# mjevans26/Satellite_ComputerVision

Hardware: AMD Instinct MI355X
Metric: tiles/sec (train) 256x256x4 U-Net (higher is better)
Workload: dtype bf16; 1 GPU; U-Net 256x256x4 bfloat16 training, batch 64 per GPU (BASELINE configs[1]); global_batch=64, parallelism=dp1, loss=weighted_categorical_crossentropy, optimizer=adam(9e-4)

## Files before the change

### include/satcv.h

```cpp
#ifndef SATCV_H
#define SATCV_H
#include <stdint.h>
#ifdef __cplusplus
extern "C" {
#endif

typedef double satcv_stat_t;

enum { SATCV_OK = 0, SATCV_ERR_INVALID = -1, SATCV_ERR_HIP = -2, SATCV_ERR_UNSUPPORTED = -3 };
enum { SATCV_F32 = 0, SATCV_BF16 = 1,
       SATCV_FP8 = 2 ,
       SATCV_FP8X = 3 ,
       SATCV_F64 = 4  };
#define SATCV_STAT_ROWS 32

const char* satcv_version(void);
const char* satcv_last_error(void);
int satcv_device_info(int32_t* out4);

int satcv_ingest_nhwc(const float* src, void* dst, int64_t npix, int32_t c, int32_t cpad,
                      int32_t dtype, void* stream);
int satcv_ingest_nhwc_scaled(const float* src, void* dst, int64_t npix, int32_t c, int32_t cpad, float mul, int32_t dtype, void* stream);
int satcv_ingest_chw(const void* src, int32_t src_kind, float scale, void* dst, int32_t n,
                     int32_t c, int32_t h, int32_t w, int32_t cpad, int32_t dtype, void* stream);
// ... 104 lines not shown
  const float* in_scale; const float* in_shift; int32_t in_relu;
  const void* w_dgrad;
  void* dx; int32_t lddx;
  float* dw; int32_t cin, cout;
  int32_t n, h, w_;
  int32_t kh, kw, dil;
  float* workspace; int64_t workspace_bytes;
  int32_t dtype;
  int32_t accumulate;
  satcv_stat_t* bst_sums; int32_t bst_sums_ld;
  const float* bst_mean; const float* bst_rstd;
  int32_t bst_act_form;
  const void* dpool; int32_t lddp; const void* amax;
  const float* hg_dlogits; const float* hg_w; int32_t hg_ncls;
  int32_t defer_reduce;
} satcv_bwdf_desc;
int64_t satcv_conv2d_bwd_fused_workspace(const satcv_bwdf_desc* d);
int satcv_conv2d_bwd_fused(const satcv_bwdf_desc* d, void* stream);
int satcv_conv2d_bwd_fused_reduce_job(const satcv_bwdf_desc* d, satcv_reduce_job* job);

typedef struct satcv_bwdf_plan_info {
  int32_t cin, cout, nw, wps, pool, nodg, cins, hg;
  int32_t bst, pad_;
  int64_t tiles, workgroups, tiles_min, tiles_max, lds_bytes, ws_bytes;
} satcv_bwdf_plan_info;
int satcv_conv2d_bwd_fused_plan_info(const satcv_bwdf_desc* d, int32_t ncu, satcv_bwdf_plan_info* info);

typedef struct satcv_ctbf_desc {
  const void* g; int32_t ldg;
  const void* yup; int32_t ldy;
// ... 385 lines not shown
```

### satellite_computervision_amd/_lib.py

```python
import ctypes as C
import os

import torch

from . import switches

_HERE = os.path.dirname(os.path.abspath(__file__))
LIB_PATH = switches.read('lib') or os.path.join(_HERE, 'libsatcv.so')

F32, BF16, FP8, FP8X, F64 = 0, 1, 2, 3, 4
STAT_ROWS = 32
COMPOSITE_MAX_T = 256

c_i32, c_i64, c_f32, c_vp = C.c_int32, C.c_int64, C.c_float, C.c_void_p


class ConvDesc(C.Structure):
    _fields_ = [('x0', c_vp), ('x1', c_vp), ('c0', c_i32), ('c1', c_i32),
                ('in_scale', c_vp), ('in_shift', c_vp), ('in_relu', c_i32),
                ('w', c_vp), ('bias', c_vp), ('y', c_vp), ('ldy', c_i32),
                ('stats', c_vp), ('stats_ld', c_i32),
                ('n', c_i32), ('h', c_i32), ('w_', c_i32),
                ('cout', c_i32), ('cout_pad', c_i32),
                ('kh', c_i32), ('kw', c_i32), ('dil', c_i32),
# ... 132 lines not shown
                   'ws': ('cin', 'nt', 'wps', 'wn', 'dil'), 'tr': ('cin', 'cout', 'th'),
                   'convt_thin': ('cin', 'cout', 'nw', 'wps', 'nsplit'), 'convt_thin_dgrad': ('cin', 'cout', 'nw', 'wps')}


class BwdfDesc(C.Structure):
    _fields_ = [('g', c_vp), ('yraw', c_vp), ('ldg', c_i32),
                ('bn_scale', c_vp), ('bn_shift', c_vp), ('bn_mean', c_vp), ('bn_rstd', c_vp), ('bn_coef', c_vp), ('linear', c_i32),
                ('x0', c_vp), ('x1', c_vp), ('c0', c_i32), ('c1', c_i32),
                ('in_scale', c_vp), ('in_shift', c_vp), ('in_relu', c_i32),
                ('w_dgrad', c_vp), ('dx', c_vp), ('lddx', c_i32),
                ('dw', c_vp), ('cin', c_i32), ('cout', c_i32),
                ('n', c_i32), ('h', c_i32), ('w_', c_i32), ('kh', c_i32), ('kw', c_i32), ('dil', c_i32),
                ('workspace', c_vp), ('workspace_bytes', c_i64), ('dtype', c_i32), ('accumulate', c_i32),
                ('bst_sums', c_vp), ('bst_sums_ld', c_i32), ('bst_mean', c_vp), ('bst_rstd', c_vp), ('bst_act_form', c_i32),
                ('dpool', c_vp), ('lddp', c_i32), ('amax', c_vp),
                ('hg_dlogits', c_vp), ('hg_w', c_vp), ('hg_ncls', c_i32), ('defer_reduce', c_i32)]


class CtbfDesc(C.Structure):
    _fields_ = [('g', c_vp), ('ldg', c_i32), ('yup', c_vp), ('ldy', c_i32),
                ('bn_scale', c_vp), ('bn_shift', c_vp), ('bn_mean', c_vp), ('bn_rstd', c_vp), ('bn_c1', c_vp), ('bn_c2', c_vp), ('linear', c_i32),
                ('x', c_vp), ('ldx', c_i32), ('in_scale', c_vp), ('in_shift', c_vp), ('in_relu', c_i32),
                ('w_dgrad', c_vp), ('w_npad', c_i32), ('dx', c_vp), ('lddx', c_i32), ('dw', c_vp), ('cin', c_i32), ('cout', c_i32),
                ('n', c_i32), ('h', c_i32), ('w_', c_i32), ('f', c_i32), ('workspace', c_vp), ('workspace_bytes', c_i64),
                ('dtype', c_i32), ('accumulate', c_i32), ('defer_reduce', c_i32),
                ('bst_sums', c_vp), ('bst_sums_ld', c_i32), ('bst_mean', c_vp), ('bst_rstd', c_vp)]


class BwdfPlanInfo(C.Structure):
    _fields_ = [(k, c_i32) for k in ('cin', 'cout', 'nw', 'wps', 'pool', 'nodg', 'cins', 'hg', 'bst', 'pad_')] + \
               [(k, c_i64) for k in ('tiles', 'workgroups', 'tiles_min', 'tiles_max', 'lds_bytes', 'ws_bytes')]
# ... 216 lines not shown
```

### satellite_computervision_amd/csrc/conv_bwd_fused.hip

```cpp
#include "igemm_common.hpp"
#include <cstdlib>
#include <cstring>

#ifndef BWDF_ABL
#define BWDF_ABL 0
#endif
#define FABL(bit) ((BWDF_ABL & (bit)) != 0)

int wgrad_reduce_slabs(const float* ws, float* dw, int nslab, int taps, int kpad, int npad, int cin, int nvalid, int accumulate, hipStream_t st);
void reduce_job_fill(satcv_reduce_job* job, const float* ws, float* dw, int nslab, int taps, int kpad, int npad, int cin, int nvalid, int transposed, int accumulate);
void satcv_prof_begin(int kind, double flops, hipStream_t st);
void satcv_prof_end(int kind, hipStream_t st);

struct BwdfArgs {
  IgemmArgs e;
  const void* g; const void* yraw; int ldg;
  const float* bn_scale; const float* bn_shift; const float* bn_mean; const float* bn_rstd; const float* bn_coef; int bn_c, linear;
  const void* x0; const void* x1; int c0, c1;
  const float* in_scale; const float* in_shift; int in_relu;
  const void* w;
  float* ws;
  int tiles_x, tiles_y;
  satcv_stat_t* bst_sums; int bst_ld; const float* bst_mean; const float* bst_rstd;
  int bst_act_form;
  const void* dp; int lddp; const unsigned char* amax;
  const float* hg_dl; const float* hg_w;
};

__device__ __forceinline__ bf16x4 tr_read4(const bf16* p) {
  short4v v = __builtin_amdgcn_ds_read_tr16_b64_v4i16((__attribute__((address_space(3))) short4v*)(p));
  return __builtin_bit_cast(bf16x4, v);
}

constexpr bool bwdf_carries_sums(bool nodg, int wps, bool pool) { return !nodg && (wps != 1 || pool); }

template <int CIN, int COUT, int NW, int WPS, bool POOL = false, bool NODG = false, int CINS = CIN, bool HG = false>
__global__ __launch_bounds__(NW * 64, WPS) void bwd_fused_kernel(const BwdfArgs a, const int total_tiles) {
  static_assert(!HG || !POOL, "the head feeds a decoder block");
  typedef bf16 T;
  constexpr int TW = 32, TH = 8, BM = 256, RL = TH + 2, CL = TW + 2, PITCH = CL, EL = 8, NTHREADS = NW * 64;
  constexpr int SD = COUT / 8, SX = CIN / 8, SXR = CINS / 8;
// ... 354 lines not shown
    }
    if (POOL && t + 1 < t_hi) issue_pool(n0, y0, x0);
    __syncthreads();
    {
      constexpr int OPITCH = CIN + 8, VPR = CIN / 8;
      T* ldsO = reinterpret_cast<T*>(smem_raw + O_OFF);
      T* op = ldsO + ((wave * MT) * 32 + 4 * hh) * OPITCH + r;
#pragma unroll
      for (int m = 0; m < MT; ++m)
#pragma unroll
        for (int n = 0; n < NT; ++n)
#pragma unroll
          for (int i = 0; i < 16; ++i) op[(m * 32 + (i & 3) + 8 * (i >> 2)) * OPITCH + n * 32] = (T)acc[m][n][i];
      __syncthreads();
      const int vq = tid % VPR;
      T* yp = reinterpret_cast<T*>(a.e.y) + ((size_t)(tn0 * a.e.h + ty0) * a.e.w_ + tx0) * a.e.ldy + vq * 8;
      const unsigned row_pitch = (unsigned)a.e.w_ * a.e.ldy;
      const T* xact = ldsX + vq * XSTRIDE;
#pragma unroll 2
      for (int it = tid; it < BM * VPR; it += NTHREADS) {
        const int q = it / VPR;
        const uint4 dv = *reinterpret_cast<const uint4*>(ldsO + q * OPITCH + vq * 8);
        if constexpr (!FABL(4)) *reinterpret_cast<uint4*>(yp + (size_t)((q / TW) * row_pitch + (q % TW) * (unsigned)a.e.ldy)) = dv;
        else asm volatile("" :: "v"(dv.x));
        if (BST && a.bst_sums) {
          const bf16x8 d8 = __builtin_bit_cast(bf16x8, dv);
          const bf16x8 a8 = *reinterpret_cast<const bf16x8*>(xact + q * EL);
#pragma unroll
          for (int e = 0; e < 8; ++e) {
            const float df = (float)d8[e], af = (float)a8[e];
            bs1[e] += af > 0.f ? df : 0.f;
            bs2[e] += df * af;
          }
        }
      }
    }
    }
    __syncthreads();
// ... 74 lines not shown
  long long grid = (long long)ncu * per_cu;
  if (grid > total) grid = total;
  return (int)grid;
}

static bool bwdf_shape_ok(const satcv_bwdf_desc* d, int& cin_s) {
  cin_s = d->c0 + d->c1;
  if (d->dtype != SATCV_BF16 || d->kh != 3 || d->kw != 3 || d->dil != 1) return false;
  if (d->n <= 0 || d->h <= 0 || d->w_ <= 0 || !satcv_pixels_ok(d->n, d->h, d->w_, 1)) return false;
  if (d->x1 && d->c0 % 8 != 0) return false;
  if (d->h % 8 != 0 || d->w_ % 32 != 0) return false;
  if (d->ldg % 8 != 0 || ((uintptr_t)d->g % 16) != 0 || ((uintptr_t)d->yraw % 16) != 0) return false;
  if (d->hg_dlogits && (!d->hg_w || d->hg_ncls != 2 || d->dpool || ((uintptr_t)d->hg_dlogits % 8) != 0)) return false;
  if (d->dx && (d->lddx % 8 != 0 || ((uintptr_t)d->dx % 16) != 0)) return false;
  if ((long long)d->w_ * d->ldg >= (1 << 23)) return false;
  if (d->dpool) {
    if (!d->amax || d->lddp % 8 != 0 || ((uintptr_t)d->dpool % 16) != 0 || ((uintptr_t)d->amax % 8) != 0 || d->x1) return false;
    if (d->dx) return cin_s == 32 && d->cin == 32 && d->cout == 64;
    return cin_s == 16 && d->cin <= 16 && d->cout == 32 && !d->bst_sums;
  }
  if (!d->dx) return false;
  if (d->bst_sums && cin_s == 64 && d->cout == 64) return false;
  if (!((cin_s == 32 && d->cout == 32) || (cin_s == 64 && d->cout == 32) || (cin_s == 64 && d->cout == 64))) return false;
  if (d->cin != cin_s) return false;
  return true;
}

template <int CIN, int COUT, int NW, int WPS, bool POOL = false, bool NODG = false, int CINS = CIN, bool HG = false>
static int bwdf_launch(const satcv_bwdf_desc* d, hipStream_t st, bool query, int64_t* ws_bytes, satcv_reduce_job* job, int ncu, satcv_bwdf_plan_info* plan) {
  using G = BwdfGeom<CIN, COUT, NW, NODG>;
// ... 13 lines not shown
  }
  if (job) { reduce_job_fill(job, d->workspace, d->dw, grid, 9, CIN, COUT, d->cin, COUT, 0, d->accumulate); return SATCV_OK; }
  if (query) { *ws_bytes = (int64_t)need; return SATCV_OK; }
  SATCV_CHECK((size_t)d->workspace_bytes >= need, "bwd_fused: workspace %lld < %zu", (long long)d->workspace_bytes, need);
  BwdfArgs a;
  memset(&a, 0, sizeof(a));
  a.e.y = d->dx; a.e.ldy = d->lddx; a.e.n = d->n; a.e.h = d->h; a.e.w_ = d->w_; a.e.cout = CIN; a.e.cout_pad = CIN; a.e.cstat = CIN;
  a.e.imgs = 1; a.e.rpi = 8; a.e.tiles_x = d->w_ / 32; a.e.tiles_y = d->h / 8; a.e.n_tiles = 1;
  a.g = d->g; a.yraw = d->yraw; a.ldg = d->ldg;
  a.bn_scale = d->bn_scale; a.bn_shift = d->bn_shift; a.bn_mean = d->bn_mean; a.bn_rstd = d->bn_rstd; a.bn_coef = d->bn_coef; a.bn_c = d->cout; a.linear = d->linear;
  a.x0 = d->x0; a.x1 = d->x1; a.c0 = d->c0; a.c1 = d->c1; a.in_scale = d->in_scale; a.in_shift = d->in_shift; a.in_relu = d->in_relu;
  a.w = d->w_dgrad; a.ws = d->workspace; a.tiles_x = d->w_ / 32; a.tiles_y = d->h / 8;
  a.bst_sums = d->bst_sums; a.bst_ld = d->bst_sums_ld; a.bst_mean = d->bst_mean; a.bst_rstd = d->bst_rstd; a.bst_act_form = d->bst_act_form;
  a.dp = d->dpool; a.lddp = d->lddp; a.amax = reinterpret_cast<const unsigned char*>(d->amax);
  a.hg_dl = d->hg_dlogits; a.hg_w = d->hg_w;
  auto kern = bwd_fused_kernel<CIN, COUT, NW, WPS, POOL, NODG, CINS, HG>;
  { const int rc = satcv_ensure_dynamic_lds(reinterpret_cast<const void*>(kern), G::LDS); if (rc) return rc; }
  const double flops = (NODG ? 2.0 : 4.0) * d->n * d->h * d->w_ * (double)CINS * COUT * 9;
  satcv_prof_begin(3, flops, st);
  hipLaunchKernelGGL(kern, dim3(grid), dim3(NW * 64), G::LDS, st, a, (int)total);
  satcv_prof_end(3, st);
  hipError_t e = hipGetLastError();
  if (e != hipSuccess) { satcv_set_error("bwd_fused launch: %s", hipGetErrorString(e)); return SATCV_ERR_HIP; }
  if (d->defer_reduce) return SATCV_OK;
  return wgrad_reduce_slabs(d->workspace, d->dw, grid, 9, CIN, COUT, d->cin, COUT, d->accumulate, st);
}

static int bwdf_dispatch(const satcv_bwdf_desc* d, hipStream_t st, bool query, int64_t* ws_bytes, satcv_reduce_job* job = nullptr, int ncu = 0,
                         satcv_bwdf_plan_info* plan = nullptr) {
  int cin_s;
// ... 42 lines not shown
```

### satellite_computervision_amd/engine.py

```python
import ctypes as C
import itertools
from collections import defaultdict, namedtuple
from fractions import Fraction

import numpy as np
import torch

from . import ops, parallel, switches
from ._lib import lib, check, F32, BF16, STAT_ROWS
from .params import FlatParams

_M16_DEFAULT = ops.options()['igemm_m16']

BN_EPS = 1e-3
BN_MOMENTUM = 0.99


class KTensor:
    _ids = itertools.count()

    def __init__(self, node, channels, down=Fraction(1), name=None):
        self.id = next(KTensor._ids)
        self.node, self.channels, self.down, self.name = node, channels, down, name

# ... 45 lines not shown
        order.append(node)
    for t in outputs:
        visit(t.node)
    return order


class TRef:

    def __init__(self, srcs, n, h, w, affine=None, relu=False):
        self.srcs, self.n, self.h, self.w = srcs, n, h, w
        self.affine, self.relu = affine, relu

    @property
    def c(self):
        return sum(c for _, c in self.srcs)


def _fp(t, off=0):
    return None if t is None else t.data_ptr() + t.element_size() * off


class Runtime(FlatParams):

    def __init__(self, model, dtype):
        if not torch.cuda.is_available():
            raise RuntimeError('satellite_computervision_amd needs a ROCm GPU (no CPU fallback)')
        super().__init__()
        self.model, self.dtype = model, dtype
        self.pack_dtype = dtype
        self.tdtype = ops.TORCH_DTYPE[dtype]
# ... 683 lines not shown
                                                               _fp(aff['rstd'], aoff), dgamma, dbeta, _fp(coef), accum, st))
        else:
            fin0 = lambda st: check(lib.satcv_bn_bwd_finalize(_fp(sums, sums_off), sums_ld, c, cnt, dgamma, dbeta, _fp(coef), accum, st))
        if self.sync_bn:
            def fin(st):
                parallel.allreduce_mean_(sums)
                if parts:
                    parallel.allreduce_mean_(act['buf'])
                fin0(st)
        else:
            fin = fin0
        app = lambda st: check(lib.satcv_bn_bwd_apply(C.byref(d), st))
        app.label = f"bn_bwd_apply n{n} {hh}x{ww} c{c} f{f}"
        app.work = dict(kind='bn_bwd_apply', px=n * hh * ww, c=c, esize=es)
        app.coef = coef
        if frozen:
            def fin_frozen(st):
                sums.zero_()
                coef.zero_()
                if act:
                    act['buf'].zero_()
            return None, fin_frozen, app
        return red, fin, app

    def ident_vecs(self, c):
        if c not in self.ident:
            self.ident[c] = (torch.ones(c, dtype=torch.float32, device=self.rt.dev), torch.zeros(c, dtype=torch.float32, device=self.rt.dev))
            self.keep.append(self.ident[c])
        return self.ident[c]

# ... 229 lines not shown
        fusable = (self.dt == ops.BF16 and da is not None and not graws and not BIAS_NOISE and cx['k'] == 3 and cx['dil'] == 1 and da[2] == cx['ldy']
                   and self.gact.get(node.inputs[0].id) is None and lay.name not in self.shared_layers)
        if fusable and dp is None and self._thin_fused(v) is not None:
            return
        dy = self._z(self.n, r.h, r.w, cout)
        bn = self.bn_bwd_steps(v.da_ptr, da[2] if da is not None else 0, dp[0].data_ptr() if dp is not None else None,
                               cout, self.gpool_f.get(tout.id, 1), cx['y'].data_ptr() + cx['yoff'] * es, cx['ldy'], cx['aff'], cx['aoff'], sums, 0, cout, cout,
                               r.h, r.w, dy.data_ptr(), cout, rt.gptr(lay.name + '/bias') if BIAS_NOISE else None,
                               rt.gptr(lay.bn_name + '/gamma'), rt.gptr(lay.bn_name + '/beta'), accum,
                               linear=0 if node.attrs.get('relu', True) else 1, frozen=lay.bn_name in self.frozen,
                               act=self.act_sums.get(tout.id) if (self.act_sums.get(tout.id) or {}).get('parts') else None)
        if fusable and dp is not None and self._pooled_fused(v, bn) is not None:
            return
        self._separate(v, bn, dy)

    def _fused_desc(self, v, coef, want_dx=True, **kw):
        rt, n, es, cx = self.rt, self.n, self.es, v.cx
        lay, r, aff, aoff, cout = v.node.layer, cx['r'], cx['aff'], cx['aoff'], cx['cout']
        pk, sa = rt.packed[lay.name], self._src_args(r)
        gin = self._z(n, r.h, r.w, r.c) if want_dx else None
        fz = ops.make_bwdf_desc(g=v.da_ptr, yraw=cx['y'].data_ptr() + cx['yoff'] * es, ldg=cx['ldy'], bn_scale=_fp(aff['scale'], aoff), bn_shift=_fp(aff['shift'], aoff),
                                bn_mean=_fp(aff['mean'], aoff), bn_rstd=_fp(aff['rstd'], aoff), bn_coef=_fp(coef),
                                w_dgrad=pk['dgrad'].data_ptr() if want_dx else None, dx=gin.data_ptr() if want_dx else None, lddx=r.c if want_dx else 0,
                                dw=rt.gptr(lay.name + '/kernel'), cin=pk['cin'], cout=cout, n=n, h=r.h, w_=r.w, dtype=self.dt, accumulate=v.accum, **kw, **sa)
        return fz, sa, gin

    def _emit_fused(self, v, fz, nb, red, fin, gin, suffix, dyparts, **work):
        n, cx, lay = self.n, v.cx, v.node.layer
        r, cout = cx['r'], cx['cout']
        self.fused_ws_need = max(self.fused_ws_need, nb)
        self.fdescs.append(fz)
        self.keep.append(fz)
        self.bwd += [fin] if (v.pre is not None or red is None) else [red, fin]
        fstep = lambda st: check(lib.satcv_conv2d_bwd_fused(C.byref(fz), st))
        fstep.label = f"bwd_fused k3 n{n} {r.h}x{r.w} {fz.c0}+{fz.c1}->{cout}{suffix}"
        fstep.work = dict(kind='bwd_fused', taps=9, px=n * r.h * r.w, cin=fz.cin, cout=cout, esize=self.es, **work)
        self.bwd.append(fstep)
        if gin is not None:
            self.set_grad(v.node.inputs[0], lay, gin, r.c)
        self.dbg['dyparts:' + lay.name] = dict(g=v.da, **{k: cx[k] for k in ('y', 'yoff', 'ldy', 'aff', 'aoff', 'cout')}, **dyparts)
        self.dbg_ctx(lay, v.da, v.dp, cx)
        return fstep

    def _thin_fused(self, v):
        node, cx = v.node, v.cx
        rt, tin, tout, lay, r, cout = self.rt, node.inputs[0], node.outputs[0], node.layer, cx['r'], cx['cout']
        if not getattr(rt.model, 'fuse_thin_bwd', True) or tin.node.op == 'input':
            return None
        cinp = r.c
        coef = self._z(2, cout, dtype=torch.float32)
        fz, sa, gin = self._fused_desc(v, coef, linear=0 if node.attrs.get('relu', True) else 1)
        sums_below = self.sums_below(fz, tin, sa, cinp)
        hf = self.head_feed.get(tout.id)
        if (hf is not None and getattr(rt.model, 'fuse_head_grad', True) and hf['ncls'] == 2 and hf['c'] == cout == 32 and cinp == 32
                and hf['fused_reduce'] and v.pre is not None and len(self.consumers.get(tout.id, [])) == 1):
            fz.hg_dlogits, fz.hg_w, fz.hg_ncls = self.dlogits.data_ptr(), hf['w'], 2
            if lib.satcv_conv2d_bwd_fused_workspace(C.byref(fz)) < 0:
                fz.hg_dlogits, fz.hg_w, fz.hg_ncls = None, None, 0
            else:
                hf['hd'].dx = None
        nbf = lib.satcv_conv2d_bwd_fused_workspace(C.byref(fz))
        if nbf < 0 and sums_below is not None:
            fz.bst_sums, fz.bst_sums_ld, fz.bst_mean, fz.bst_rstd = None, 0, None, None
            sums_below = None
            nbf = lib.satcv_conv2d_bwd_fused_workspace(C.byref(fz))
        if nbf < 0:
            return None
        if sums_below is not None:
            self.fused[tin.id] = sums_below
        red, fin, _ = self.bn_bwd_steps(v.da_ptr, v.da[2], None, 0, 1, cx['y'].data_ptr() + cx['yoff'] * self.es, cx['ldy'], cx['aff'], cx['aoff'], v.sums, 0,
                                        cout, cout, r.h, r.w, None, 0, None, rt.gptr(lay.bn_name + '/gamma'), rt.gptr(lay.bn_name + '/beta'), v.accum,
                                        linear=fz.linear, frozen=lay.bn_name in self.frozen, coef=coef)
        dyparts = dict(coef=coef, linear=fz.linear)
        if fz.hg_dlogits:
            dyparts['head'] = (self.dlogits, hf['wname'])
        return self._emit_fused(v, fz, nbf, red, fin, gin, f"{' +bnred' if fz.bst_sums else ''}{' +headgrad' if fz.hg_dlogits else ''}", dyparts)

    def _pooled_fused(self, v, bn):
        node, dp = v.node, v.dp
        rt, tin, tout, lay = self.rt, node.inputs[0], node.outputs[0], node.layer
        red, fin, app = bn
        amax = self.amax_of.get(tout.id)
        if (amax is None or not getattr(rt.model, 'fuse_pool_bwd', True) or self.gpool_f.get(tout.id, 1) != 2 or dp[1] != 0
                or lay.bn_name in self.frozen):
            return None
        want_dx = tin.node.op != 'input'
        cinp = v.cx['r'].c
        fzp, sa, ginp = self._fused_desc(v, app.coef, want_dx, linear=0, dpool=dp[0].data_ptr(), lddp=dp[2], amax=amax.data_ptr())
        ent = None
        if (want_dx and self.POOL_SUMS and tin.node.op == 'pool' and len(self.consumers[tin.id]) == 1 and sa['in_scale'] is None
                and len(self.vals[tin.id].srcs) == 1 and tin.node.inputs[0].channels == cinp):
# ... 48 lines not shown
        if g is None:
            return
        off = 0
        for t in node.inputs:
            self.gact[t.id] = (g[0], g[1] + off, g[2])
            off += t.channels

    def pool(self, node, cx):
        tin, tout = node.inputs[0], node.outputs[0]
        if tout.id in self.gact:
            if self.gact[tout.id][1] != 0:
                raise NotImplementedError('pooled gradient in a channel slice')
            self.gpool[tin.id] = self.gact[tout.id]
            self.gpool_f[tin.id] = cx['f']

    def concat_bn_relu(self, node, cx):
        rt, n, dt, es, consumers = self.rt, self.n, self.dt, self.es, self.consumers
        ta, tb = node.inputs
        tout = node.outputs[0]
        g = self.gact.get(tout.id)
        if g is None:
            return
        ra, rb, aff, ca, cb = cx['ra'], cx['rb'], cx['aff'], cx['ca'], cx['cb']
        ctot = ca + cb
        hh, ww = ra.h, ra.w
        pre = self.fused.get(tout.id)
        sums = pre if pre is not None else self._z(STAT_ROWS, 2, ctot, dtype=torch.float64)
        dskip = self._z(n, hh, ww, ca)
        du = self._z(n, hh, ww, cb)
        bn = node.layer.name
        upl = tb.node.layer
        if g[2] != ctot:
            raise NotImplementedError('decoder concat gradient in a channel slice')
        gptr_ = g[0].data_ptr() + g[1] * es
        if not (tb.node.op == 'convT' and BIAS_NOISE) and ca % 8 == 0:
            sec = dict(yraw1=rb.srcs[0][0].data_ptr(), ldy1=cb, dy1=du.data_ptr(), lddy1=cb, c_split=ca)
            ctbf = None
            cxt = self.ctx.get(id(tb.node)) if tb.node.op == 'convT' else None
            if (CTBF and dt == ops.BF16 and cxt is not None and bn not in self.frozen and upl.name not in self.shared_layers and cxt['f'] == 2
                    and cb in CTBF_COUTS and len(consumers.get(tb.id, [])) == 1):
                rT = cxt['r']
                saT = self._src_args(rT)
                probe = ops.make_ctbf_desc(g=gptr_ + ca * es, ldg=ctot, yup=rb.srcs[0][0].data_ptr(), ldy=cb, bn_scale=None, bn_shift=None, bn_mean=None,
                                           bn_rstd=None, bn_c1=None, bn_c2=None, x=saT['x0'], ldx=saT['c0'], w_dgrad=rt.packed[upl.name]['dgrad'].data_ptr(),
                                           w_npad=rup(rT.c, 32), dx=saT['x0'], lddx=rT.c, dw=rt.gptr(upl.name + '/kernel'), cin=rT.c, cout=cb, n=n,
                                           h=rT.h, w_=rT.w, dtype=dt)
                if saT['x1'] is None and saT['c0'] == rT.c == rt.packed[upl.name]['cin'] and lib.satcv_convt_bwd_fused_workspace(C.byref(probe)) > 0:
                    ctbf = dict(g=gptr_ + ca * es, ldg=ctot, yup=rb.srcs[0][0].data_ptr(), ldy=cb, aff=aff, aoff=ca, ctot=ctot)
                    sec['dy1'] = None
            ent = None
            if (bn not in self.frozen and ta.id not in self.gact and any(cn.op == 'pool' for cn in consumers[ta.id])
                    and len([cn for cn in consumers[ta.id] if cn.op != 'pool']) == 1 and ta.channels == ca):
                ent = self.act_sums_for(ta)
            if ent is not None:
                sec.update(sk_sums=_fp(ent['buf']), sk_sums_ld=ca)
                ent['parts'].add('skip')
            r_, f_, a_ = self.bn_bwd_steps(gptr_, ctot, None, 0, 1, ra.srcs[0][0].data_ptr(), ca, aff, 0, sums, 0, ctot, ctot, hh, ww,
                                           dskip.data_ptr(), ca, None, rt.gptr(bn + '/gamma'), rt.gptr(bn + '/beta'), frozen=bn in self.frozen,
                                           second=sec)
            if ent is not None:
                a_.label += ' +skipsums'
            if ctbf is not None:
                a_.label += ' (skip half)'
                a_.work = dict(kind='bn_bwd_apply', px=n * hh * ww, c=ca, esize=es)
                ctbf['coef'] = a_.coef
            self.bwd += [f_, a_] if (pre is not None or r_ is None) else [r_, f_, a_]
            self.graw[tb.id] = ctbf if ctbf is not None else du
        else:
            ra_, fa_, aa_ = self.bn_bwd_steps(gptr_, ctot, None, 0, 1, ra.srcs[0][0].data_ptr(), ca, aff, 0, sums, 0, ctot, ca, hh, ww,
                                              dskip.data_ptr(), ca, None, rt.gptr(bn + '/gamma'), rt.gptr(bn + '/beta'), frozen=bn in self.frozen)
            rb_, fb_, ab_ = self.bn_bwd_steps(gptr_ + ca * es, ctot, None, 0, 1, rb.srcs[0][0].data_ptr(), cb, aff, ca, sums, ca, ctot, cb,
                                              hh, ww, du.data_ptr(), cb, rt.gptr(upl.name + '/bias') if (tb.node.op == 'convT' and BIAS_NOISE) else None,
                                              rt.gptr(bn + '/gamma') + 4 * ca, rt.gptr(bn + '/beta') + 4 * ca, frozen=bn in self.frozen)
            self.bwd += [fa_, fb_, aa_, ab_] if (pre is not None or ra_ is None) else [ra_, rb_, fa_, fb_, aa_, ab_]
            self.graw[tb.id] = du
        self.gact[ta.id] = (dskip, 0, ca)
        self.dbg['dskip:' + bn] = dskip
        self.dbg['du:' + bn] = du
# ... 16 lines not shown
                                    x=sa['x0'], ldx=sa['c0'], in_scale=sa['in_scale'], in_shift=sa['in_shift'], in_relu=sa['in_relu'],
                                    w_dgrad=pk['dgrad'].data_ptr(), w_npad=rup(cinp, 32), dx=gin.data_ptr(), lddx=cinp, dw=rt.gptr(lay.name + '/kernel'),
                                    cin=cinp, cout=cout, n=n, h=r.h, w_=r.w, dtype=dt)
            sums_below = self.sums_below(fz, tin, sa, cinp)
            if sums_below is not None:
                self.fused[tin.id] = sums_below
            nbc = lib.satcv_convt_bwd_fused_workspace(C.byref(fz))
            if nbc <= 0:
                raise RuntimeError('convt_bwd_fused: the probe accepted this shape, the final descriptor did not')
            wsc = self._z(max(nbc // 4, 1), dtype=torch.float32)
            fz.workspace, fz.workspace_bytes = wsc.data_ptr(), nbc
            self.keep.append(fz)
            cstep = lambda st: check(lib.satcv_convt_bwd_fused(C.byref(fz), st))
            cstep.label = f"convt_bwd_fused n{n} {r.h}x{r.w} {cinp}<-4x{cout}{' +bnred' if fz.bst_sums else ''}"
            cstep.work = dict(kind='convt_bwd_fused', px=n * r.h * r.w, cin=cinp, cout=cout, esize=self.es)
            self.bwd.append(cstep)
        else:
            self.bwd.append(self.wgrad_step(r, du.data_ptr(), cout, lay, pk['cin'], cout, r.h, r.w, 1, 1, f=f))
            self.bwd.append(self.dgrad_step(tin, x0=du.data_ptr(), c0=cout, w=pk['dgrad'].data_ptr(), y=gin.data_ptr(), ldy=cinp, n=n, h=r.h,
                                            w_=r.w, cout=cinp, cout_pad=rup(cinp, 32), kh=1, kw=1, dil=1, mode_in=1, f=f, dtype=dt))
        self.set_grad(tin, lay, gin, cinp)
```

### satellite_computervision_amd/model_tools.py

```python
import ctypes as C
import json
import os
from collections import defaultdict
from fractions import Fraction

import numpy as np
import torch

from . import engine as E
from . import ops, switches
from ._lib import lib, check, F32, BF16
from .training import (LossSpec, _LossArg, weighted_categorical_crossentropy, weighted_bce, gen_dice, iou_loss, mse_4d,
                       Adam, SGD, RMSprop, resolve_optimizer, reset_slots_on_recompile, apply_optimizer, MeanIoU, History,
                       ModelCheckpoint, LearningRateScheduler, ReduceLROnPlateau, EarlyStopping, TensorBoard, run_callbacks,
                       record_callback_logs, resolve_loss, metric_from_confusion, fit_loop)

_DEFAULT_DTYPE = 'bfloat16'
_RNG = np.random.default_rng(0)
_UIDS = defaultdict(int)


def set_compute_dtype(name):
    global _DEFAULT_DTYPE
    assert name in ('bfloat16', 'float32')
# ... 526 lines not shown
                subs = [l for l in (lay, node.attrs['owner'].bn_layer) if l is not None]
            for l in subs:
                if id(l) not in seen:
                    seen.add(id(l))
                    self.layers.append(l)
                    self.param_specs += l.specs
        self.compute_dtype = dtype or _DEFAULT_DTYPE
        self.bn_bessel = True
        self.fuse_head_bn_bwd = switches.read('fuse_head_bn_bwd')
        self.fuse_dgrad_bn_bwd = switches.read('fuse_dgrad_bn_bwd') != 0
        self.wgrad_side_stream = switches.read('wgrad_stream')
        self.fuse_pool_bn_sums = switches.read('fuse_pool_bn_sums')
        self.fuse_head_grad = switches.read('fuse_head_grad')
        self.fuse_pool_bwd = switches.read('fuse_pool_bwd')
        self.fuse_thin_bwd = switches.read('fuse_thin_bwd')
        self.sync_bn = switches.read('sync_bn')
        self._rt = None
        self.optimizer, self._loss, self._metrics = None, None, []
        self.metrics_names = []
        self.stop_training = False
        self._builder = None
        self.output_names = [t.name for t in self.outputs]

    @property
    def runtime(self):
        if self._rt is None:
            self._rt = E.Runtime(self, BF16 if self.compute_dtype == 'bfloat16' else F32)
            if self.optimizer is not None:
                self.optimizer._rt = self._rt
                self._rt.adam_state[0:1].fill_(self.optimizer._lr)
# ... 659 lines not shown
```

### satellite_computervision_amd/ops.py

```python
import ctypes as C
import itertools

import torch

from . import _lib
from ._lib import lib, check, ConvDesc, WgradDesc, BnBwdDesc, HeadDesc, F32, BF16, FP8, FP8X, STAT_ROWS

TORCH_DTYPE = {F32: torch.float32, BF16: torch.bfloat16, FP8: torch.float8_e4m3fn, FP8X: torch.float8_e4m3fn}
DTYPE_CODE = {torch.float32: F32, torch.bfloat16: BF16, torch.float8_e4m3fn: FP8}


def rup(a, b):
    return (a + b - 1) // b * b


def stream_ptr():
    return C.c_void_p(torch.cuda.current_stream().cuda_stream)


def ptr(t):
    if t is None:
        return None
    assert t.is_cuda, 'satcv ops need device tensors (no CPU fallback)'
    return C.c_void_p(t.data_ptr())
# ... 153 lines not shown
    d = WgradDesc()
    d.x0, d.x1, d.c0, d.c1 = x0, x1, c0, c1
    d.in_scale, d.in_shift, d.in_relu = in_scale, in_shift, int(in_relu)
    d.dy, d.lddy, d.dw, d.cin, d.cout = dy, lddy, dw, cin, cout
    d.n, d.h, d.w_, d.kh, d.kw, d.dil = n, h, w_, kh, kw, dil
    d.mode_dy, d.f, d.transposed = mode_dy, f, transposed
    d.workspace, d.workspace_bytes, d.dtype, d.accumulate = workspace, workspace_bytes, dtype, int(accumulate)
    d.whole_chip = int(whole_chip)
    d.defer_reduce = int(defer_reduce)
    return d


def make_bwdf_desc(*, g, yraw, ldg, bn_scale, bn_shift, bn_mean, bn_rstd, bn_coef, x0, c0, w_dgrad, dx, lddx, dw, cin, cout, n, h, w_, dtype,
                   linear=0, x1=None, c1=0, in_scale=None, in_shift=None, in_relu=0, kh=3, kw=3, dil=1, workspace=None, workspace_bytes=0,
                   accumulate=0, bst_sums=None, bst_sums_ld=0, bst_mean=None, bst_rstd=None, bst_act_form=0, dpool=None, lddp=0, amax=None,
                   hg_dlogits=None, hg_w=None, hg_ncls=0, defer_reduce=0):
    from ._lib import BwdfDesc
    d = BwdfDesc()
    d.g, d.yraw, d.ldg = g, yraw, ldg
    d.bn_scale, d.bn_shift, d.bn_mean, d.bn_rstd, d.bn_coef, d.linear = bn_scale, bn_shift, bn_mean, bn_rstd, bn_coef, int(linear)
    d.x0, d.x1, d.c0, d.c1 = x0, x1, c0, c1
    d.in_scale, d.in_shift, d.in_relu = in_scale, in_shift, int(in_relu)
    d.w_dgrad, d.dx, d.lddx, d.dw, d.cin, d.cout = w_dgrad, dx, lddx, dw, cin, cout
    d.n, d.h, d.w_, d.kh, d.kw, d.dil = n, h, w_, kh, kw, dil
    d.workspace, d.workspace_bytes, d.dtype, d.accumulate = workspace, workspace_bytes, dtype, int(accumulate)
    d.bst_sums, d.bst_sums_ld, d.bst_mean, d.bst_rstd, d.bst_act_form = bst_sums, bst_sums_ld, bst_mean, bst_rstd, int(bst_act_form)
    d.dpool, d.lddp, d.amax = dpool, lddp, amax
    d.hg_dlogits, d.hg_w, d.hg_ncls = hg_dlogits, hg_w, int(hg_ncls)
    d.defer_reduce = int(defer_reduce)
    return d


def conv_bwd_fused(g, yraw, scale, shift, mean, rstd, coef, x, w_dgrad, cin, cout, *, x1=None, in_scale=None, in_shift=None, in_relu=False,
                   linear=False, accumulate_into=None, bst=None, dpool=None, amax=None, want_dx=True, head=None):
    n, h, w_, c0 = x.shape
    c1 = x1.shape[-1] if x1 is not None else 0
    dx = torch.empty(n, h, w_, c0 + c1, dtype=x.dtype, device=x.device) if want_dx else None
    dw = accumulate_into if accumulate_into is not None else torch.empty(3, 3, cin, cout, dtype=torch.float32, device=x.device)
    d = make_bwdf_desc(g=_p(g), yraw=_p(yraw), ldg=g.shape[-1] if g is not None else yraw.shape[-1], bn_scale=_p(scale), bn_shift=_p(shift), bn_mean=_p(mean), bn_rstd=_p(rstd),
                       bn_coef=_p(coef), x0=_p(x), c0=c0, x1=_p(x1), c1=c1, in_scale=_p(in_scale), in_shift=_p(in_shift), in_relu=in_relu,
                       w_dgrad=_p(w_dgrad), dx=_p(dx), lddx=c0 + c1, dw=_p(dw), cin=cin, cout=cout, n=n, h=h, w_=w_, dtype=DTYPE_CODE[x.dtype],
                       linear=linear, accumulate=accumulate_into is not None, dpool=_p(dpool), lddp=dpool.shape[-1] if dpool is not None else 0,
                       amax=_p(amax), **(dict(hg_dlogits=_p(head[0]), hg_w=_p(head[1]), hg_ncls=head[0].shape[-1]) if head else {}),
                       **(dict(bst_sums=_p(bst['sums']), bst_sums_ld=bst['sums'].shape[-1], bst_mean=_p(bst.get('mean')), bst_rstd=_p(bst.get('rstd')),
# ... 260 lines not shown
```

Before: 8310 tiles/s.

## Write fused conv dgrad into separate concat gradient planes for thin decoder layers

Adds a second output plane (dx1) to the fused conv backward kernel. Input-gradient channels past c0 are now written to a separate contiguous tensor instead of one interleaved concat-width buffer. The engine uses this for thin concat_bn_relu inputs whose halves are under 128 bytes per pixel, so the downstream BN-backward apply and the fused transposed-conv backward read dense per-half gradients rather than strided slices. The intent is better memory coalescing for narrow channel slices. In exchange it adds a per-thread branch on the store address and another path through the graph planner, which raises an error if the promised consumers are not fused.

After: 8382 tiles/s, median of 6. Within noise of the previous version (+0.9%).

```diff
diff --git a/include/satcv.h b/include/satcv.h
--- a/include/satcv.h
+++ b/include/satcv.h
@@ -142,6 +142,7 @@
   const void* dpool; int32_t lddp; const void* amax;
   const float* hg_dlogits; const float* hg_w; int32_t hg_ncls;
   int32_t defer_reduce;
+  void* dx1; int32_t lddx1;
 } satcv_bwdf_desc;
 int64_t satcv_conv2d_bwd_fused_workspace(const satcv_bwdf_desc* d);
 int satcv_conv2d_bwd_fused(const satcv_bwdf_desc* d, void* stream);
diff --git a/satellite_computervision_amd/_lib.py b/satellite_computervision_amd/_lib.py
--- a/satellite_computervision_amd/_lib.py
+++ b/satellite_computervision_amd/_lib.py
@@ -170,7 +170,8 @@
                 ('workspace', c_vp), ('workspace_bytes', c_i64), ('dtype', c_i32), ('accumulate', c_i32),
                 ('bst_sums', c_vp), ('bst_sums_ld', c_i32), ('bst_mean', c_vp), ('bst_rstd', c_vp), ('bst_act_form', c_i32),
                 ('dpool', c_vp), ('lddp', c_i32), ('amax', c_vp),
-                ('hg_dlogits', c_vp), ('hg_w', c_vp), ('hg_ncls', c_i32), ('defer_reduce', c_i32)]
+                ('hg_dlogits', c_vp), ('hg_w', c_vp), ('hg_ncls', c_i32), ('defer_reduce', c_i32),
+                ('dx1', c_vp), ('lddx1', c_i32)]
 
 
 class CtbfDesc(C.Structure):
diff --git a/satellite_computervision_amd/csrc/conv_bwd_fused.hip b/satellite_computervision_amd/csrc/conv_bwd_fused.hip
--- a/satellite_computervision_amd/csrc/conv_bwd_fused.hip
+++ b/satellite_computervision_amd/csrc/conv_bwd_fused.hip
@@ -25,6 +25,7 @@
   int bst_act_form;
   const void* dp; int lddp; const unsigned char* amax;
   const float* hg_dl; const float* hg_w;
+  void* dx1; int lddx1;
 };
 
 __device__ __forceinline__ bf16x4 tr_read4(const bf16* p) {
@@ -409,14 +410,16 @@
           for (int i = 0; i < 16; ++i) op[(m * 32 + (i & 3) + 8 * (i >> 2)) * OPITCH + n * 32] = (T)acc[m][n][i];
       __syncthreads();
       const int vq = tid % VPR;
-      T* yp = reinterpret_cast<T*>(a.e.y) + ((size_t)(tn0 * a.e.h + ty0) * a.e.w_ + tx0) * a.e.ldy + vq * 8;
-      const unsigned row_pitch = (unsigned)a.e.w_ * a.e.ldy;
+      const bool plane1 = !POOL && a.dx1 != nullptr && vq * 8 >= a.c0;
+      const unsigned ldo = plane1 ? (unsigned)a.lddx1 : (unsigned)a.e.ldy;
+      T* yp = (plane1 ? reinterpret_cast<T*>(a.dx1) + (vq * 8 - a.c0) : reinterpret_cast<T*>(a.e.y) + vq * 8) + ((size_t)(tn0 * a.e.h + ty0) * a.e.w_ + tx0) * ldo;
+      const unsigned row_pitch = (unsigned)a.e.w_ * ldo;
       const T* xact = ldsX + vq * XSTRIDE;
 #pragma unroll 2
       for (int it = tid; it < BM * VPR; it += NTHREADS) {
         const int q = it / VPR;
         const uint4 dv = *reinterpret_cast<const uint4*>(ldsO + q * OPITCH + vq * 8);
-        if constexpr (!FABL(4)) *reinterpret_cast<uint4*>(yp + (size_t)((q / TW) * row_pitch + (q % TW) * (unsigned)a.e.ldy)) = dv;
+        if constexpr (!FABL(4)) *reinterpret_cast<uint4*>(yp + (size_t)((q / TW) * row_pitch + (q % TW) * ldo)) = dv;
         else asm volatile("" :: "v"(dv.x));
         if (BST && a.bst_sums) {
           const bf16x8 d8 = __builtin_bit_cast(bf16x8, dv);
@@ -521,6 +524,7 @@
   if (d->hg_dlogits && (!d->hg_w || d->hg_ncls != 2 || d->dpool || ((uintptr_t)d->hg_dlogits % 8) != 0)) return false;
   if (d->dx && (d->lddx % 8 != 0 || ((uintptr_t)d->dx % 16) != 0)) return false;
   if ((long long)d->w_ * d->ldg >= (1 << 23)) return false;
+  if (d->dx1 && (!d->x1 || !d->dx || d->dpool || ((uintptr_t)d->dx1 % 16) != 0 || d->lddx1 % 8 != 0 || d->lddx1 < d->c1 || d->lddx < d->c0)) return false;
   if (d->dpool) {
     if (!d->amax || d->lddp % 8 != 0 || ((uintptr_t)d->dpool % 16) != 0 || ((uintptr_t)d->amax % 8) != 0 || d->x1) return false;
     if (d->dx) return cin_s == 32 && d->cin == 32 && d->cout == 64;
@@ -564,6 +568,7 @@
   a.bst_sums = d->bst_sums; a.bst_ld = d->bst_sums_ld; a.bst_mean = d->bst_mean; a.bst_rstd = d->bst_rstd; a.bst_act_form = d->bst_act_form;
   a.dp = d->dpool; a.lddp = d->lddp; a.amax = reinterpret_cast<const unsigned char*>(d->amax);
   a.hg_dl = d->hg_dlogits; a.hg_w = d->hg_w;
+  a.dx1 = d->dx1; a.lddx1 = d->lddx1;
   auto kern = bwd_fused_kernel<CIN, COUT, NW, WPS, POOL, NODG, CINS, HG>;
   { const int rc = satcv_ensure_dynamic_lds(reinterpret_cast<const void*>(kern), G::LDS); if (rc) return rc; }
   const double flops = (NODG ? 2.0 : 4.0) * d->n * d->h * d->w_ * (double)CINS * COUT * 9;
diff --git a/satellite_computervision_amd/engine.py b/satellite_computervision_amd/engine.py
--- a/satellite_computervision_amd/engine.py
+++ b/satellite_computervision_amd/engine.py
@@ -83,6 +83,24 @@
     @property
     def c(self):
         return sum(c for _, c in self.srcs)
+
+
+class GradPlanes:
+
+    def __init__(self, a, b):
+        self.a, self.b = a, b
+
+    def cat(self):
+        return torch.cat([self.a, self.b], dim=-1)
+
+    def double(self):
+        return self.cat().double()
+
+    def float(self):
+        return self.cat().float()
+
+    def clone(self):
+        return self.cat()
 
 
 def _fp(t, off=0):
@@ -796,6 +814,7 @@
         app.label = f"bn_bwd_apply n{n} {hh}x{ww} c{c} f{f}"
         app.work = dict(kind='bn_bwd_apply', px=n * hh * ww, c=c, esize=es)
         app.coef = coef
+        app.desc = d
         if frozen:
             def fin_frozen(st):
                 sums.zero_()
@@ -1055,14 +1074,15 @@
             return
         self._separate(v, bn, dy)
 
-    def _fused_desc(self, v, coef, want_dx=True, **kw):
+    def _fused_desc(self, v, coef, want_dx=True, alloc_dx=True, **kw):
         rt, n, es, cx = self.rt, self.n, self.es, v.cx
         lay, r, aff, aoff, cout = v.node.layer, cx['r'], cx['aff'], cx['aoff'], cx['cout']
         pk, sa = rt.packed[lay.name], self._src_args(r)
-        gin = self._z(n, r.h, r.w, r.c) if want_dx else None
+        gin = self._z(n, r.h, r.w, r.c) if (want_dx and alloc_dx) else None
+        dxp = (gin.data_ptr() if alloc_dx else sa['x0']) if want_dx else None
         fz = ops.make_bwdf_desc(g=v.da_ptr, yraw=cx['y'].data_ptr() + cx['yoff'] * es, ldg=cx['ldy'], bn_scale=_fp(aff['scale'], aoff), bn_shift=_fp(aff['shift'], aoff),
                                 bn_mean=_fp(aff['mean'], aoff), bn_rstd=_fp(aff['rstd'], aoff), bn_coef=_fp(coef),
-                                w_dgrad=pk['dgrad'].data_ptr() if want_dx else None, dx=gin.data_ptr() if want_dx else None, lddx=r.c if want_dx else 0,
+                                w_dgrad=pk['dgrad'].data_ptr() if want_dx else None, dx=dxp, lddx=r.c if want_dx else 0,
                                 dw=rt.gptr(lay.name + '/kernel'), cin=pk['cin'], cout=cout, n=n, h=r.h, w_=r.w, dtype=self.dt, accumulate=v.accum, **kw, **sa)
         return fz, sa, gin
 
@@ -1076,6 +1096,7 @@
         fstep = lambda st: check(lib.satcv_conv2d_bwd_fused(C.byref(fz), st))
         fstep.label = f"bwd_fused k3 n{n} {r.h}x{r.w} {fz.c0}+{fz.c1}->{cout}{suffix}"
         fstep.work = dict(kind='bwd_fused', taps=9, px=n * r.h * r.w, cin=fz.cin, cout=cout, esize=self.es, **work)
+        fstep.desc = fz
         self.bwd.append(fstep)
         if gin is not None:
             self.set_grad(v.node.inputs[0], lay, gin, r.c)
@@ -1090,7 +1111,7 @@
             return None
         cinp = r.c
         coef = self._z(2, cout, dtype=torch.float32)
-        fz, sa, gin = self._fused_desc(v, coef, linear=0 if node.attrs.get('relu', True) else 1)
+        fz, sa, _ = self._fused_desc(v, coef, alloc_dx=False, linear=0 if node.attrs.get('relu', True) else 1)
         sums_below = self.sums_below(fz, tin, sa, cinp)
         hf = self.head_feed.get(tout.id)
         if (hf is not None and getattr(rt.model, 'fuse_head_grad', True) and hf['ncls'] == 2 and hf['c'] == cout == 32 and cinp == 32
@@ -1109,13 +1130,41 @@
             return None
         if sums_below is not None:
             self.fused[tin.id] = sums_below
+        gin = self._thin_dx(fz, tin, r, sums_below is not None)
         red, fin, _ = self.bn_bwd_steps(v.da_ptr, v.da[2], None, 0, 1, cx['y'].data_ptr() + cx['yoff'] * self.es, cx['ldy'], cx['aff'], cx['aoff'], v.sums, 0,
                                         cout, cout, r.h, r.w, None, 0, None, rt.gptr(lay.bn_name + '/gamma'), rt.gptr(lay.bn_name + '/beta'), v.accum,
                                         linear=fz.linear, frozen=lay.bn_name in self.frozen, coef=coef)
         dyparts = dict(coef=coef, linear=fz.linear)
         if fz.hg_dlogits:
             dyparts['head'] = (self.dlogits, hf['wname'])
-        return self._emit_fused(v, fz, nbf, red, fin, gin, f"{' +bnred' if fz.bst_sums else ''}{' +headgrad' if fz.hg_dlogits else ''}", dyparts)
+        planes = dict(dx_planes=1) if fz.dx1 else {}
+        return self._emit_fused(v, fz, nbf, red, fin, gin, f"{' +bnred' if fz.bst_sums else ''}{' +headgrad' if fz.hg_dlogits else ''}{' dx-planes' if planes else ''}",
+                                dyparts, **planes)
+
+    def _thin_dx(self, fz, tin, r, carries_sums):
+        n = self.n
+        pl = self.concat_planes(tin) if carries_sums else None
+        if pl is not None and (fz.c0, fz.c1) == pl and fz.x1:
+            ca, cb = pl
+            fz.lddx, fz.dx1, fz.lddx1 = ca, fz.dx, cb
+            if lib.satcv_conv2d_bwd_fused_workspace(C.byref(fz)) >= 0:
+                gin = GradPlanes(self._z(n, r.h, r.w, ca), self._z(n, r.h, r.w, cb))
+                fz.dx, fz.dx1 = gin.a.data_ptr(), gin.b.data_ptr()
+                return gin
+            fz.lddx, fz.dx1, fz.lddx1 = r.c, None, 0
+        gin = self._z(n, r.h, r.w, r.c)
+        fz.dx = gin.data_ptr()
+        return gin
+
+    def concat_planes(self, tcat):
+        P = tcat.node
+        if not getattr(self.rt.model, 'concat_grad_planes', True) or P.op != 'concat_bn_relu':
+            return None
+        pc = self.ctx.get(id(P))
+        ca, cb = pc['ca'], pc['cb']
+        if min(ca, cb) * self.es >= 128:
+            return None
+        return (ca, cb) if self.concat_ctbf(P, pc, pc['rb'].srcs[0][0].data_ptr(), cb) is not None else None
 
     def _pooled_fused(self, v, bn):
         node, dp = v.node, v.dp
@@ -1194,6 +1243,27 @@
             self.gpool[tin.id] = self.gact[tout.id]
             self.gpool_f[tin.id] = cx['f']
 
+    def concat_ctbf(self, node, cx, gup, ldg):
+        rt, n, dt, consumers = self.rt, self.n, self.dt, self.consumers
+        ta, tb = node.inputs
+        rb, aff, ca, cb = cx['rb'], cx['aff'], cx['ca'], cx['cb']
+        bn, upl = node.layer.name, tb.node.layer
+        if (tb.node.op == 'convT' and BIAS_NOISE) or ca % 8:
+            return None
+        cxt = self.ctx.get(id(tb.node)) if tb.node.op == 'convT' else None
+        if not (CTBF and dt == ops.BF16 and cxt is not None and bn not in self.frozen and upl.name not in self.shared_layers and cxt['f'] == 2
+                and cb in CTBF_COUTS and len(consumers.get(tb.id, [])) == 1):
+            return None
+        rT = cxt['r']
+        saT = self._src_args(rT)
+        probe = ops.make_ctbf_desc(g=gup, ldg=ldg, yup=rb.srcs[0][0].data_ptr(), ldy=cb, bn_scale=None, bn_shift=None, bn_mean=None,
+                                   bn_rstd=None, bn_c1=None, bn_c2=None, x=saT['x0'], ldx=saT['c0'], w_dgrad=rt.packed[upl.name]['dgrad'].data_ptr(),
+                                   w_npad=rup(rT.c, 32), dx=saT['x0'], lddx=rT.c, dw=rt.gptr(upl.name + '/kernel'), cin=rT.c, cout=cb, n=n,
+                                   h=rT.h, w_=rT.w, dtype=dt)
+        if saT['x1'] is None and saT['c0'] == rT.c == rt.packed[upl.name]['cin'] and lib.satcv_convt_bwd_fused_workspace(C.byref(probe)) > 0:
+            return dict(g=gup, ldg=ldg, yup=rb.srcs[0][0].data_ptr(), ldy=cb, aff=aff, aoff=ca, ctot=ca + cb)
+        return None
+
     def concat_bn_relu(self, node, cx):
         rt, n, dt, es, consumers = self.rt, self.n, self.dt, self.es, self.consumers
         ta, tb = node.inputs
@@ -1212,22 +1282,20 @@
         upl = tb.node.layer
         if g[2] != ctot:
             raise NotImplementedError('decoder concat gradient in a channel slice')
-        gptr_ = g[0].data_ptr() + g[1] * es
+        planes = g[0] if isinstance(g[0], GradPlanes) else None
+        if planes is not None:
+            gptr_, ldg_, gup = planes.a.data_ptr(), ca, planes.b.data_ptr()
+            ldgup = cb
+        else:
+            gptr_, ldg_ = g[0].data_ptr() + g[1] * es, ctot
+            gup, ldgup = gptr_ + ca * es, ctot
+        ctbf = self.concat_ctbf(node, cx, gup, ldgup)
+        if planes is not None and (ctbf is None or pre is None):
+            raise RuntimeError('concat gradient planes: the producer was promised the skip-half apply and the fused transposed-conv backward')
         if not (tb.node.op == 'convT' and BIAS_NOISE) and ca % 8 == 0:
             sec = dict(yraw1=rb.srcs[0][0].data_ptr(), ldy1=cb, dy1=du.data_ptr(), lddy1=cb, c_split=ca)
-            ctbf = None
-            cxt = self.ctx.get(id(tb.node)) if tb.node.op == 'convT' else None
-            if (CTBF and dt == ops.BF16 and cxt is not None and bn not in self.frozen and upl.name not in self.shared_layers and cxt['f'] == 2
-                    and cb in CTBF_COUTS and len(consumers.get(tb.id, [])) == 1):
-                rT = cxt['r']
-                saT = self._src_args(rT)
-                probe = ops.make_ctbf_desc(g=gptr_ + ca * es, ldg=ctot, yup=rb.srcs[0][0].data_ptr(), ldy=cb, bn_scale=None, bn_shift=None, bn_mean=None,
-                                           bn_rstd=None, bn_c1=None, bn_c2=None, x=saT['x0'], ldx=saT['c0'], w_dgrad=rt.packed[upl.name]['dgrad'].data_ptr(),
-                                           w_npad=rup(rT.c, 32), dx=saT['x0'], lddx=rT.c, dw=rt.gptr(upl.name + '/kernel'), cin=rT.c, cout=cb, n=n,
-                                           h=rT.h, w_=rT.w, dtype=dt)
-                if saT['x1'] is None and saT['c0'] == rT.c == rt.packed[upl.name]['cin'] and lib.satcv_convt_bwd_fused_workspace(C.byref(probe)) > 0:
-                    ctbf = dict(g=gptr_ + ca * es, ldg=ctot, yup=rb.srcs[0][0].data_ptr(), ldy=cb, aff=aff, aoff=ca, ctot=ctot)
-                    sec['dy1'] = None
+            if ctbf is not None:
+                sec['dy1'] = None
             ent = None
             if (bn not in self.frozen and ta.id not in self.gact and any(cn.op == 'pool' for cn in consumers[ta.id])
                     and len([cn for cn in consumers[ta.id] if cn.op != 'pool']) == 1 and ta.channels == ca):
@@ -1235,13 +1303,13 @@
             if ent is not None:
                 sec.update(sk_sums=_fp(ent['buf']), sk_sums_ld=ca)
                 ent['parts'].add('skip')
-            r_, f_, a_ = self.bn_bwd_steps(gptr_, ctot, None, 0, 1, ra.srcs[0][0].data_ptr(), ca, aff, 0, sums, 0, ctot, ctot, hh, ww,
+            r_, f_, a_ = self.bn_bwd_steps(gptr_, ldg_, None, 0, 1, ra.srcs[0][0].data_ptr(), ca, aff, 0, sums, 0, ctot, ctot, hh, ww,
                                            dskip.data_ptr(), ca, None, rt.gptr(bn + '/gamma'), rt.gptr(bn + '/beta'), frozen=bn in self.frozen,
                                            second=sec)
             if ent is not None:
                 a_.label += ' +skipsums'
             if ctbf is not None:
-                a_.label += ' (skip half)'
+                a_.label += ' (skip half)' + (' planes' if planes is not None else '')
                 a_.work = dict(kind='bn_bwd_apply', px=n * hh * ww, c=ca, esize=es)
                 ctbf['coef'] = a_.coef
             self.bwd += [f_, a_] if (pre is not None or r_ is None) else [r_, f_, a_]
@@ -1288,6 +1356,7 @@
             cstep = lambda st: check(lib.satcv_convt_bwd_fused(C.byref(fz), st))
             cstep.label = f"convt_bwd_fused n{n} {r.h}x{r.w} {cinp}<-4x{cout}{' +bnred' if fz.bst_sums else ''}"
             cstep.work = dict(kind='convt_bwd_fused', px=n * r.h * r.w, cin=cinp, cout=cout, esize=self.es)
+            cstep.desc = fz
             self.bwd.append(cstep)
         else:
             self.bwd.append(self.wgrad_step(r, du.data_ptr(), cout, lay, pk['cin'], cout, r.h, r.w, 1, 1, f=f))
diff --git a/satellite_computervision_amd/model_tools.py b/satellite_computervision_amd/model_tools.py
--- a/satellite_computervision_amd/model_tools.py
+++ b/satellite_computervision_amd/model_tools.py
@@ -564,6 +564,7 @@
         self.fuse_head_grad = switches.read('fuse_head_grad')
         self.fuse_pool_bwd = switches.read('fuse_pool_bwd')
         self.fuse_thin_bwd = switches.read('fuse_thin_bwd')
+        self.concat_grad_planes = True
         self.sync_bn = switches.read('sync_bn')
         self._rt = None
         self.optimizer, self._loss, self._metrics = None, None, []
diff --git a/satellite_computervision_amd/ops.py b/satellite_computervision_amd/ops.py
--- a/satellite_computervision_amd/ops.py
+++ b/satellite_computervision_amd/ops.py
@@ -191,7 +191,7 @@
 def make_bwdf_desc(*, g, yraw, ldg, bn_scale, bn_shift, bn_mean, bn_rstd, bn_coef, x0, c0, w_dgrad, dx, lddx, dw, cin, cout, n, h, w_, dtype,
                    linear=0, x1=None, c1=0, in_scale=None, in_shift=None, in_relu=0, kh=3, kw=3, dil=1, workspace=None, workspace_bytes=0,
                    accumulate=0, bst_sums=None, bst_sums_ld=0, bst_mean=None, bst_rstd=None, bst_act_form=0, dpool=None, lddp=0, amax=None,
-                   hg_dlogits=None, hg_w=None, hg_ncls=0, defer_reduce=0):
+                   hg_dlogits=None, hg_w=None, hg_ncls=0, defer_reduce=0, dx1=None, lddx1=0):
     from ._lib import BwdfDesc
     d = BwdfDesc()
     d.g, d.yraw, d.ldg = g, yraw, ldg
@@ -205,6 +205,7 @@
     d.dpool, d.lddp, d.amax = dpool, lddp, amax
     d.hg_dlogits, d.hg_w, d.hg_ncls = hg_dlogits, hg_w, int(hg_ncls)
     d.defer_reduce = int(defer_reduce)
+    d.dx1, d.lddx1 = dx1, lddx1
     return d
 
 
```
